# nyuolab/OmniBioTE

Measured on AMD Instinct MI355X. Metric: MLM train tokens/sec, small (8L/1024d) ctx=1024 at 1/2/4/8 MI355X, higher is better.
Workload: dtype bf16

## Files before the change

omnibiote_amd/csrc/elementwise.hip:

```cpp
#include "common.h"
#include <stdlib.h>

namespace {

template <bool INVERSE>
__global__ __launch_bounds__(256) void rope_kernel(bf16* __restrict__ qkv, const float* __restrict__ cos_t,
                                                    const float* __restrict__ sin_t, int64_t rows, int64_t T, int C, int hs) {
    const int chunks_per_row = 2 * C / 8;
    const int64_t total = rows * chunks_per_row;
    for (int64_t i = (int64_t)blockIdx.x * blockDim.x + threadIdx.x; i < total; i += (int64_t)gridDim.x * blockDim.x) {
        const int64_t row = i / chunks_per_row;
        const int col = (int)(i % chunks_per_row) * 8;
        const int d = col % hs;
        const int64_t t = row % T;
        bf16* ptr = qkv + row * 3 * C + col;
        const bf16x8 v = *reinterpret_cast<const bf16x8*>(ptr);
        const f32x4 c = *reinterpret_cast<const f32x4*>(cos_t + t * (hs / 2) + d / 2);
        const f32x4 s = *reinterpret_cast<const f32x4*>(sin_t + t * (hs / 2) + d / 2);
        bf16x8 o;
#pragma unroll
        for (int j = 0; j < 4; ++j) {
            const float xe = bf2f(v[2 * j]), xo = bf2f(v[2 * j + 1]);
            const float sj = INVERSE ? -s[j] : s[j];
            o[2 * j] = f2bf(xe * c[j] - xo * sj);
// ... 20 lines not shown
            for (int jj = 0; jj < 4; ++jj) {
                const uint32_t bits = drop_pair_bits(rk, (uint32_t)(c >> 1) + jj);
#pragma unroll
                for (int e = 0; e < 2; ++e) v[2 * jj + e] = drop_keep_bits(bits, (uint32_t)e, dc) ? f2bf(bf2f(v[2 * jj + e]) * dc.scale) : f2bf(0.f);
            }
        }
        *reinterpret_cast<bf16x8*>(out + r * cols + c) = v;
    }
}

__global__ __launch_bounds__(256) void dropout_kernel(const bf16* in, bf16* out, int64_t n8, int64_t cols, DropCfg dc) {
    for (int64_t i = (int64_t)blockIdx.x * blockDim.x + threadIdx.x; i < n8; i += (int64_t)gridDim.x * blockDim.x) {
        bf16x8 v = reinterpret_cast<const bf16x8*>(in)[i];
        const int64_t row = (i * 8) / cols;
        const uint32_t c = (uint32_t)((i * 8) - row * cols);
        const uint32_t rk = drop_rowkey((uint64_t)row, dc);
        for (int jj = 0; jj < 4; ++jj) {
            const uint32_t bits = drop_pair_bits(rk, (c >> 1) + jj);
#pragma unroll
            for (int e = 0; e < 2; ++e) v[2 * jj + e] = drop_keep_bits(bits, (uint32_t)e, dc) ? f2bf(bf2f(v[2 * jj + e]) * dc.scale) : f2bf(0.f);
        }
        reinterpret_cast<bf16x8*>(out)[i] = v;
    }
}

constexpr int EMB_CHUNK = 32;

template <bool ACC>
__device__ __forceinline__ void embed_store_row(bf16* dst, const float (&acc)[8]) {
    bf16x8 o;
#pragma unroll
    for (int j = 0; j < 8; ++j) o[j] = f2bf(acc[j]);
    if (ACC) {
        const bf16x8 old = *reinterpret_cast<const bf16x8*>(dst);
#pragma unroll
        for (int j = 0; j < 8; ++j) o[j] = f2bf(bf2f(old[j]) + bf2f(o[j]));
    }
    *reinterpret_cast<bf16x8*>(dst) = o;
}
template <bool ACC>
__device__ __forceinline__ void embed_store_row(float* dst, const float (&acc)[8]) {
    f32x4 lo = f32x4{acc[0], acc[1], acc[2], acc[3]}, hi = f32x4{acc[4], acc[5], acc[6], acc[7]};
    if (ACC) {
        lo += *reinterpret_cast<const f32x4*>(dst);
        hi += *reinterpret_cast<const f32x4*>(dst + 4);
    }
    *reinterpret_cast<f32x4*>(dst) = lo;
    *reinterpret_cast<f32x4*>(dst + 4) = hi;
}

template <bool ACC, class DST = bf16>
__global__ __launch_bounds__(128) void embed_bwd_chunk_kernel(const int64_t* __restrict__ idx, const int32_t* __restrict__ order,
                                                               const bf16* __restrict__ dout, DST* __restrict__ dwte,
                                                               float* __restrict__ slab, int64_t rows, int cols, int64_t vocab, DropCfg dc) {
    __shared__ int32_t s_row[EMB_CHUNK];
    __shared__ int64_t s_tok[EMB_CHUNK + 2];
    const int64_t c = blockIdx.x;
    const int64_t p0 = c * EMB_CHUNK;
    const int n = (int)((rows - p0) < EMB_CHUNK ? (rows - p0) : EMB_CHUNK);
    if (threadIdx.x < n) {
        const int32_t r = order[p0 + threadIdx.x];
        s_row[threadIdx.x] = r;
        s_tok[threadIdx.x + 1] = clamp_tok(idx[r], vocab);
    }
    if (threadIdx.x == 64) s_tok[0] = p0 > 0 ? clamp_tok(idx[order[p0 - 1]], vocab) : -1;
    if (threadIdx.x == 65) s_tok[n + 1] = (p0 + n < rows) ? clamp_tok(idx[order[p0 + n]], vocab) : -1;
    __syncthreads();
    const bool left_open = s_tok[0] == s_tok[1];
    const bool right_open = s_tok[n + 1] == s_tok[n];
    for (int col = threadIdx.x * 8; col < cols; col += 128 * 8) {
        float acc[8];
#pragma unroll
        for (int j = 0; j < 8; ++j) acc[j] = 0.f;
        int seg_start = 0;
        for (int i = 0; i < n; ++i) {
            const bf16x8 v = *reinterpret_cast<const bf16x8*>(dout + (int64_t)s_row[i] * cols + col);
            if (dc.thresh16) {
                const uint32_t rk = drop_rowkey((uint64_t)s_row[i], dc);
                for (int jj = 0; jj < 4; ++jj) {
                    const uint32_t bits = drop_pair_bits(rk, (uint32_t)(col >> 1) + jj);
#pragma unroll
                    for (int e = 0; e < 2; ++e)
                        if (drop_keep_bits(bits, (uint32_t)e, dc)) acc[2 * jj + e] += bf2f(f2bf(bf2f(v[2 * jj + e]) * dc.scale));
                }
            } else {
#pragma unroll
                for (int j = 0; j < 8; ++j) acc[j] += bf2f(v[j]);
            }
            const bool seg_end = (i == n - 1) || (s_tok[i + 2] != s_tok[i + 1]);
            if (seg_end) {
                const bool is_first = seg_start == 0, is_last = i == n - 1;
                if ((is_first && left_open) || (is_last && right_open)) {
                    float* dst = slab + ((c * 2 + (is_first ? 0 : 1)) * cols + col);
                    *reinterpret_cast<f32x4*>(dst) = f32x4{acc[0], acc[1], acc[2], acc[3]};
                    *reinterpret_cast<f32x4*>(dst + 4) = f32x4{acc[4], acc[5], acc[6], acc[7]};
                } else {
                    embed_store_row<ACC>(dwte + s_tok[i + 1] * cols + col, acc);
                }
#pragma unroll
                for (int j = 0; j < 8; ++j) acc[j] = 0.f;
                seg_start = i + 1;
            }
        }
    }
}

template <bool ACC, class DST = bf16>
__global__ __launch_bounds__(128) void embed_bwd_span_kernel(const int64_t* __restrict__ idx, const int32_t* __restrict__ order,
                                                              DST* __restrict__ dwte, const float* __restrict__ slab,
                                                              int64_t rows, int cols, int64_t nchunks, int64_t vocab) {
    const int64_t c = blockIdx.x;
    const int64_t p0 = c * EMB_CHUNK;
    const int64_t p1 = (p0 + EMB_CHUNK < rows) ? p0 + EMB_CHUNK : rows;
    const int64_t first = clamp_tok(idx[order[p0]], vocab), last = clamp_tok(idx[order[p1 - 1]], vocab);
    const bool single = first == last;
    const bool left_open = p0 > 0 && clamp_tok(idx[order[p0 - 1]], vocab) == first;
    const bool right_open = p1 < rows && clamp_tok(idx[order[p1]], vocab) == last;
    if (!right_open || (single && left_open)) return;
    const int slot0 = single ? 0 : 1;
    for (int col = threadIdx.x * 8; col < cols; col += 128 * 8) {
        float acc[8];
        const float* src = slab + ((c * 2 + slot0) * cols + col);
#pragma unroll
        for (int j = 0; j < 8; ++j) acc[j] = src[j];
        for (int64_t cc = c + 1; cc < nchunks; ++cc) {
            const int64_t q0 = cc * EMB_CHUNK;
            const int64_t q1 = (q0 + EMB_CHUNK < rows) ? q0 + EMB_CHUNK : rows;
            if (clamp_tok(idx[order[q0]], vocab) != last) break;
            const float* s2 = slab + ((cc * 2) * cols + col);
#pragma unroll
            for (int j = 0; j < 8; ++j) acc[j] += s2[j];
            if (clamp_tok(idx[order[q1 - 1]], vocab) != last) break;
        }
        embed_store_row<ACC>(dwte + last * cols + col, acc);
    }
}

__global__ __launch_bounds__(256) void acc32_add_kernel(float* __restrict__ acc32, const bf16* __restrict__ src, bf16* __restrict__ out,
                                                         int64_t n8, int mode) {
    for (int64_t i = (int64_t)blockIdx.x * 256 + threadIdx.x; i < n8; i += (int64_t)gridDim.x * 256) {
        float v[8];
        if (src) {
            const bf16x8 sv = *reinterpret_cast<const bf16x8*>(src + i * 8);
#pragma unroll
            for (int j = 0; j < 8; ++j) v[j] = bf2f(sv[j]);
        } else {
#pragma unroll
            for (int j = 0; j < 8; ++j) v[j] = 0.f;
        }
        if (mode != OBTE_ACC32_FIRST) {
            const f32x4 lo = *reinterpret_cast<const f32x4*>(acc32 + i * 8), hi = *reinterpret_cast<const f32x4*>(acc32 + i * 8 + 4);
#pragma unroll
            for (int j = 0; j < 4; ++j) { v[j] += lo[j]; v[4 + j] += hi[j]; }
        }
        if (src || mode == OBTE_ACC32_FIRST) {
            *reinterpret_cast<f32x4*>(acc32 + i * 8) = f32x4{v[0], v[1], v[2], v[3]};
            *reinterpret_cast<f32x4*>(acc32 + i * 8 + 4) = f32x4{v[4], v[5], v[6], v[7]};
        }
        if (mode == OBTE_ACC32_LAST) {
            bf16x8 o;
#pragma unroll
            for (int j = 0; j < 8; ++j) o[j] = f2bf(v[j]);
            *reinterpret_cast<bf16x8*>(out + i * 8) = o;
        }
    }
}

__global__ __launch_bounds__(256) void masked_ce_kernel(const bf16* __restrict__ logits, const int64_t* __restrict__ target,
                                                         const uint8_t* __restrict__ mlm_mask, const uint8_t* __restrict__ prev_mask,
                                                         const float* __restrict__ grad_scale, float row_scale,
                                                         float* __restrict__ row_loss, bf16* __restrict__ dlogits, int64_t vocab,
                                                         const int64_t* __restrict__ row_index, const float* __restrict__ row_scale_vec) {
    __shared__ float red[8];
    const int64_t r = blockIdx.x;
    const int64_t src = row_index ? row_index[r] : r;
    const int lane = threadIdx.x & 63, wave = threadIdx.x >> 6;
    bf16* drow = dlogits + r * vocab;
    if (!row_index && mlm_mask && !mlm_mask[r]) {
        if (threadIdx.x == 0 && row_loss) row_loss[r] = 0.f;
        if (prev_mask && !prev_mask[r]) return;
        const bf16x8 z = {};
        for (int64_t c = (int64_t)threadIdx.x * 8; c < vocab; c += 256 * 8) *reinterpret_cast<bf16x8*>(drow + c) = z;
        return;
    }
    const bf16* lrow = logits + src * vocab;
    float m = -INFINITY, l = 0.f;
    for (int64_t c = (int64_t)threadIdx.x * 8; c < vocab; c += 256 * 8) {
// ... 446 lines not shown

extern "C" int obte_embedding_fwd_dropout(const int64_t* idx, const obte_bf16* wte, obte_bf16* out, int64_t rows, int cols,
                                          int64_t vocab, float p, uint64_t seed, obte_stream s) {
    OBTE_REQUIRE(idx && wte && out, "obte_embedding_fwd: null pointer");
    OBTE_REQUIRE(rows >= 0 && cols > 0 && cols % 8 == 0 && vocab > 0, "obte_embedding_fwd: cols must be a multiple of 8");
    if (check_p("obte_embedding_fwd", p)) return OBTE_EINVAL;
    if (rows == 0) return OBTE_OK;
    hipLaunchKernelGGL(embed_fwd_kernel, dim3(stream_grid(rows * (cols / 8), 256)), dim3(256), 0, (hipStream_t)s, idx,
                       (const bf16*)wte, (bf16*)out, rows, cols, vocab, make_drop(p, seed, OBTE_SITE_EMBED));
    OBTE_CHECK_LAUNCH("obte_embedding_fwd");
    return OBTE_OK;
}

extern "C" int obte_embedding_fwd(const int64_t* idx, const obte_bf16* wte, obte_bf16* out, int64_t rows, int cols,
                                  int64_t vocab, obte_stream s) {
    return obte_embedding_fwd_dropout(idx, wte, out, rows, cols, vocab, 0.f, 0, s);
}

__global__ __launch_bounds__(256) void dropout_rows_kernel(const bf16* __restrict__ in, const bf16* __restrict__ aux, bf16* __restrict__ out,
                                                           const int64_t* __restrict__ rows, int64_t n_rows, int cols, DropCfg cfg) {
    const int64_t i = (int64_t)blockIdx.x * 4 + (threadIdx.x >> 6);
    if (i >= n_rows) return;
    const int lane = threadIdx.x & 63;
    const uint32_t rk = drop_rowkey((uint64_t)rows[i], cfg);
    for (int c = lane * 8; c < cols; c += 512) {
        bf16x8 v = *reinterpret_cast<const bf16x8*>(in + i * cols + c);
        bf16x8 a = {};
        if (aux) a = *reinterpret_cast<const bf16x8*>(aux + i * cols + c);
#pragma unroll
        for (int jj = 0; jj < 4; ++jj) {
            const uint32_t bits = drop_pair_bits(rk, ((uint32_t)c >> 1) + jj);
#pragma unroll
            for (int e = 0; e < 2; ++e) {
                const int j = 2 * jj + e;
                const float t = drop_keep_bits(bits, (uint32_t)e, cfg) ? bf2f(f2bf(bf2f(v[j]) * cfg.scale)) : 0.f;
                v[j] = aux ? f2bf(bf2f(a[j]) + t) : f2bf(t);
            }
        }
        *reinterpret_cast<bf16x8*>(out + i * cols + c) = v;
    }
}

extern "C" int obte_dropout_bf16(const obte_bf16* in, obte_bf16* out, int64_t n, int64_t cols, float p, uint64_t seed, int32_t site,
                                 obte_stream s) {
    OBTE_REQUIRE(in && out && n > 0 && n % 8 == 0, "obte_dropout_bf16: null pointer or n not a positive multiple of 8");
    OBTE_REQUIRE(cols > 0 && cols % 8 == 0 && n % cols == 0 && cols < (1ll << 32), "obte_dropout_bf16: cols must be a multiple of 8 that divides n");
    if (check_p("obte_dropout_bf16", p)) return OBTE_EINVAL;
    hipLaunchKernelGGL(dropout_kernel, dim3(stream_grid(n / 8, 256)), dim3(256), 0, (hipStream_t)s, (const bf16*)in, (bf16*)out, n / 8,
                       cols, make_drop(p, seed, (uint32_t)site));
    OBTE_CHECK_LAUNCH("obte_dropout_bf16");
    return OBTE_OK;
}

extern "C" int64_t obte_embedding_bwd_ws_bytes(int64_t rows, int cols) {
    return cdiv64(rows, EMB_CHUNK) * 2 * (int64_t)cols * (int64_t)sizeof(float);
}

extern "C" int obte_embedding_bwd_dropout(const int64_t* idx, const int32_t* order, const obte_bf16* dout, obte_bf16* dwte,
                                          void* ws, int64_t rows, int cols, int64_t vocab, int accumulate, float p, uint64_t seed,
                                          obte_stream s) {
    OBTE_REQUIRE(idx && order && dout && dwte && ws, "obte_embedding_bwd: null pointer");
    if (check_p("obte_embedding_bwd", p)) return OBTE_EINVAL;
    const DropCfg dc = make_drop(p, seed, OBTE_SITE_EMBED);
    OBTE_REQUIRE(rows > 0 && cols > 0 && cols % 8 == 0 && vocab > 0, "obte_embedding_bwd: bad shape");
    OBTE_REQUIRE(rows < (1ll << 31), "obte_embedding_bwd: too many rows");
    hipStream_t st = (hipStream_t)s;
    if (!accumulate && hipMemsetAsync(dwte, 0, (size_t)vocab * cols * sizeof(obte_bf16), st) != hipSuccess) {
        obte_set_error("obte_embedding_bwd: memset failed");
        return OBTE_ELAUNCH;
    }
    const int64_t nchunks = cdiv64(rows, EMB_CHUNK);
    if (accumulate)
        hipLaunchKernelGGL(embed_bwd_chunk_kernel<true>, dim3((unsigned)nchunks), dim3(128), 0, st, idx, order, (const bf16*)dout,
                           (bf16*)dwte, (float*)ws, rows, cols, vocab, dc);
    else
        hipLaunchKernelGGL(embed_bwd_chunk_kernel<false>, dim3((unsigned)nchunks), dim3(128), 0, st, idx, order, (const bf16*)dout,
                           (bf16*)dwte, (float*)ws, rows, cols, vocab, dc);
    OBTE_CHECK_LAUNCH("obte_embedding_bwd(chunk)");
    if (accumulate)
        hipLaunchKernelGGL(embed_bwd_span_kernel<true>, dim3((unsigned)nchunks), dim3(128), 0, st, idx, order, (bf16*)dwte,
                           (const float*)ws, rows, cols, nchunks, vocab);
    else
        hipLaunchKernelGGL(embed_bwd_span_kernel<false>, dim3((unsigned)nchunks), dim3(128), 0, st, idx, order, (bf16*)dwte,
                           (const float*)ws, rows, cols, nchunks, vocab);
    OBTE_CHECK_LAUNCH("obte_embedding_bwd(span)");
    return OBTE_OK;
}

extern "C" int obte_acc32_add_bf16(float* acc32, const obte_bf16* src, obte_bf16* out, int64_t n, int mode, obte_stream s) {
    OBTE_REQUIRE(acc32 && n > 0 && n % 8 == 0, "obte_acc32_add_bf16: null buffer or n not a positive multiple of 8");
    OBTE_REQUIRE(mode >= OBTE_ACC32_FIRST && mode <= OBTE_ACC32_LAST && (mode != OBTE_ACC32_LAST || out), "obte_acc32_add_bf16: bad mode, or LAST without out");
    if (!src && mode == OBTE_ACC32_MORE) return OBTE_OK;
    hipLaunchKernelGGL(acc32_add_kernel, dim3(stream_grid(n / 8, 256)), dim3(256), 0, (hipStream_t)s, acc32, (const bf16*)src, (bf16*)out, n / 8, mode);
    OBTE_CHECK_LAUNCH("obte_acc32_add_bf16");
    return OBTE_OK;
}

extern "C" int obte_embedding_bwd_acc32(const int64_t* idx, const int32_t* order, const obte_bf16* dout, float* acc32, obte_bf16* dwte,
                                        void* ws, int64_t rows, int cols, int64_t vocab, int mode, float p, uint64_t seed, obte_stream s) {
    OBTE_REQUIRE(idx && order && dout && acc32 && ws, "obte_embedding_bwd_acc32: null pointer");
    OBTE_REQUIRE(mode >= OBTE_ACC32_FIRST && mode <= OBTE_ACC32_LAST && (mode != OBTE_ACC32_LAST || dwte), "obte_embedding_bwd_acc32: bad mode, or LAST without dwte");
    if (check_p("obte_embedding_bwd_acc32", p)) return OBTE_EINVAL;
    const DropCfg dc = make_drop(p, seed, OBTE_SITE_EMBED);
    OBTE_REQUIRE(rows > 0 && cols > 0 && cols % 8 == 0 && vocab > 0, "obte_embedding_bwd_acc32: bad shape");
    OBTE_REQUIRE(rows < (1ll << 31), "obte_embedding_bwd_acc32: too many rows");
    hipStream_t st = (hipStream_t)s;
    const bool first = mode == OBTE_ACC32_FIRST;
    if (first && hipMemsetAsync(acc32, 0, (size_t)vocab * cols * sizeof(float), st) != hipSuccess) {
        obte_set_error("obte_embedding_bwd_acc32: memset failed");
        return OBTE_ELAUNCH;
    }
    const int64_t nchunks = cdiv64(rows, EMB_CHUNK);
    if (first)
        hipLaunchKernelGGL((embed_bwd_chunk_kernel<false, float>), dim3((unsigned)nchunks), dim3(128), 0, st, idx, order, (const bf16*)dout, acc32, (float*)ws,
                           rows, cols, vocab, dc);
    else
        hipLaunchKernelGGL((embed_bwd_chunk_kernel<true, float>), dim3((unsigned)nchunks), dim3(128), 0, st, idx, order, (const bf16*)dout, acc32, (float*)ws,
                           rows, cols, vocab, dc);
    OBTE_CHECK_LAUNCH("obte_embedding_bwd_acc32(chunk)");
    if (first)
        hipLaunchKernelGGL((embed_bwd_span_kernel<false, float>), dim3((unsigned)nchunks), dim3(128), 0, st, idx, order, acc32, (const float*)ws, rows, cols,
                           nchunks, vocab);
    else
        hipLaunchKernelGGL((embed_bwd_span_kernel<true, float>), dim3((unsigned)nchunks), dim3(128), 0, st, idx, order, acc32, (const float*)ws, rows, cols,
                           nchunks, vocab);
    OBTE_CHECK_LAUNCH("obte_embedding_bwd_acc32(span)");
    if (mode == OBTE_ACC32_LAST) return obte_acc32_add_bf16(acc32, nullptr, dwte, vocab * (int64_t)cols, OBTE_ACC32_LAST, s);
    return OBTE_OK;
}

extern "C" int obte_embedding_bwd_acc(const int64_t* idx, const int32_t* order, const obte_bf16* dout, obte_bf16* dwte,
                                      void* ws, int64_t rows, int cols, int64_t vocab, int accumulate, obte_stream s) {
    return obte_embedding_bwd_dropout(idx, order, dout, dwte, ws, rows, cols, vocab, accumulate, 0.f, 0, s);
}

extern "C" int obte_embedding_bwd(const int64_t* idx, const int32_t* order, const obte_bf16* dout, obte_bf16* dwte,
                                  void* ws, int64_t rows, int cols, int64_t vocab, obte_stream s) {
    return obte_embedding_bwd_dropout(idx, order, dout, dwte, ws, rows, cols, vocab, 0, 0.f, 0, s);
}

extern "C" int obte_masked_ce_fwd_bwd_reuse(const obte_bf16* logits, const int64_t* target, const uint8_t* mlm_mask,
                                            const uint8_t* prev_mask, const float* grad_scale, float row_scale, float* row_loss,
                                            obte_bf16* dlogits, int64_t rows, int64_t vocab, obte_stream s) {
    OBTE_REQUIRE(logits && target && mlm_mask && grad_scale && dlogits, "obte_masked_ce_fwd_bwd: null pointer");
    OBTE_REQUIRE(rows > 0 && rows < (1ll << 31) && vocab > 0 && vocab % 8 == 0, "obte_masked_ce_fwd_bwd: vocab must be a multiple of 8");
    hipLaunchKernelGGL(masked_ce_kernel, dim3((unsigned)rows), dim3(256), 0, (hipStream_t)s, (const bf16*)logits, target, mlm_mask,
                       prev_mask, grad_scale, row_scale, row_loss, (bf16*)dlogits, vocab, (const int64_t*)nullptr, (const float*)nullptr);
    OBTE_CHECK_LAUNCH("obte_masked_ce_fwd_bwd");
    return OBTE_OK;
}

namespace {
__global__ __launch_bounds__(256) void rows_copy_kernel(const bf16* __restrict__ src, const int64_t* __restrict__ rows, bf16* __restrict__ dst,
                                                         int64_t n_rows, int64_t total_rows, int cols, int scatter) {
    const int wave = threadIdx.x >> 6, lane = threadIdx.x & 63;
    const int64_t i = (int64_t)blockIdx.x * 4 + wave;
    if (i >= n_rows) return;
    int64_t r = rows[i];
    r = r < 0 ? 0 : (r >= total_rows ? total_rows - 1 : r);
    const bf16* s = src + (scatter ? i : r) * cols;
    bf16* d = dst + (scatter ? r : i) * cols;
    for (int c = lane * 8; c < cols; c += 64 * 8) *reinterpret_cast<bf16x8*>(d + c) = *reinterpret_cast<const bf16x8*>(s + c);
}
}
extern "C" int obte_rows_gather_bf16(const obte_bf16* src, const int64_t* rows, obte_bf16* dst, int64_t n_rows, int64_t total_rows, int32_t cols, obte_stream s) {
    OBTE_REQUIRE(src && rows && dst, "obte_rows_gather_bf16: null pointer");
    OBTE_REQUIRE(n_rows > 0 && total_rows > 0 && cols > 0 && cols % 8 == 0, "obte_rows_gather_bf16: need n_rows, total_rows > 0 and cols %% 8 == 0");
    hipLaunchKernelGGL(rows_copy_kernel, dim3((unsigned)cdiv64(n_rows, 4)), dim3(256), 0, (hipStream_t)s, (const bf16*)src, rows, (bf16*)dst, n_rows, total_rows, cols, 0);
    OBTE_CHECK_LAUNCH("obte_rows_gather_bf16");
    return OBTE_OK;
}
extern "C" int obte_rows_scatter_bf16(const obte_bf16* src, const int64_t* rows, obte_bf16* dst, int64_t n_rows, int64_t total_rows, int32_t cols, obte_stream s) {
    OBTE_REQUIRE(src && rows && dst, "obte_rows_scatter_bf16: null pointer");
    OBTE_REQUIRE(n_rows > 0 && n_rows <= total_rows && cols > 0 && cols % 8 == 0, "obte_rows_scatter_bf16: need 0 < n_rows <= total_rows and cols %% 8 == 0");
    if (hipMemsetAsync(dst, 0, (size_t)total_rows * cols * 2, (hipStream_t)s) != hipSuccess) { obte_set_error("obte_rows_scatter_bf16: memset failed"); return OBTE_ELAUNCH; }
    hipLaunchKernelGGL(rows_copy_kernel, dim3((unsigned)cdiv64(n_rows, 4)), dim3(256), 0, (hipStream_t)s, (const bf16*)src, rows, (bf16*)dst, n_rows, total_rows, cols, 1);
    OBTE_CHECK_LAUNCH("obte_rows_scatter_bf16");
    return OBTE_OK;
}
// ... 236 lines not shown
```

omnibiote_amd/csrc/layernorm.hip:

```cpp
#include "common.h"
#include <stdlib.h>

namespace {

constexpr int LN_BWD_MAX_BLOCKS = 512;

template <int NCH, bool FULL>
__global__ __launch_bounds__(256) void ln_fwd_kernel(const bf16* __restrict__ x, const bf16* __restrict__ w,
                                                      bf16* __restrict__ y, float* __restrict__ mean,
                                                      float* __restrict__ rstd, int64_t rows, int cols, float eps) {
    const int wave = __builtin_amdgcn_readfirstlane(threadIdx.x >> 6), lane = threadIdx.x & 63;
    const int64_t row = (int64_t)blockIdx.x * 4 + wave;
    if (row >= rows) return;
    const bf16* xr = x + row * cols;
    float v[NCH][8];
    bf16x8 wq[NCH];
    float sum = 0.f;
    if (FULL) {
        bf16x8 t[NCH];
#pragma unroll
        for (int i = 0; i < NCH; ++i) t[i] = *reinterpret_cast<const bf16x8*>(xr + (lane + 64 * i) * 8);
#pragma unroll
        for (int i = 0; i < NCH; ++i) wq[i] = *reinterpret_cast<const bf16x8*>(w + (lane + 64 * i) * 8);
        __builtin_amdgcn_sched_barrier(0);
#pragma unroll
        for (int i = 0; i < NCH; ++i)
#pragma unroll
            for (int j = 0; j < 8; ++j) { v[i][j] = bf2f(t[i][j]); sum += v[i][j]; }
    } else {
#pragma unroll
        for (int i = 0; i < NCH; ++i) {
            const int c = (lane + 64 * i) * 8;
            if (c < cols) {
                const bf16x8 t = *reinterpret_cast<const bf16x8*>(xr + c);
#pragma unroll
                for (int j = 0; j < 8; ++j) { v[i][j] = bf2f(t[j]); sum += v[i][j]; }
            } else {
#pragma unroll
                for (int j = 0; j < 8; ++j) v[i][j] = 0.f;
            }
        }
    }
    const float mu = (FULL ? wave_sum_dpp(sum) : wave_sum(sum)) / (float)cols;
    float sq = 0.f;
#pragma unroll
    for (int i = 0; i < NCH; ++i) {
        const int c = (lane + 64 * i) * 8;
        if (FULL || c < cols) {
#pragma unroll
            for (int j = 0; j < 8; ++j) { const float d = v[i][j] - mu; sq += d * d; }
        }
    }
    const float rs = 1.0f / sqrtf((FULL ? wave_sum_dpp(sq) : wave_sum(sq)) / (float)cols + eps);
    if (lane == 0) { mean[row] = mu; rstd[row] = rs; }
    bf16* yr = y + row * cols;
#pragma unroll
    for (int i = 0; i < NCH; ++i) {
        const int c = (lane + 64 * i) * 8;
        if (FULL || c < cols) {
            const bf16x8 wv = FULL ? wq[i] : *reinterpret_cast<const bf16x8*>(w + c);
            bf16x8 o;
#pragma unroll
            for (int j = 0; j < 8; ++j) o[j] = f2bf((v[i][j] - mu) * rs * bf2f(wv[j]));
            *reinterpret_cast<bf16x8*>(yr + c) = o;
        }
    }
}

template <int NCH, bool HAS_RESID>
__global__ __launch_bounds__(256) void ln_bwd_kernel(const bf16* __restrict__ dy, const bf16* __restrict__ x,
                                                      const bf16* __restrict__ w, const float* __restrict__ mean,
                                                      const float* __restrict__ rstd, const bf16* __restrict__ dresid,
                                                      bf16* __restrict__ dx, float* __restrict__ ws, int64_t rows, int cols, int ws_accumulate) {
    extern __shared__ __attribute__((aligned(16))) char smem_raw[];
    float* red = reinterpret_cast<float*>(smem_raw);
    const int wave = threadIdx.x >> 6, lane = threadIdx.x & 63;
    float wv[NCH][8], dwacc[NCH][8];
#pragma unroll
    for (int i = 0; i < NCH; ++i) {
        const int c = (lane + 64 * i) * 8;
        bf16x8 t = {};
        if (c < cols) t = *reinterpret_cast<const bf16x8*>(w + c);
#pragma unroll
        for (int j = 0; j < 8; ++j) { wv[i][j] = bf2f(t[j]); dwacc[i][j] = 0.f; }
    }
    const float inv_c = 1.0f / (float)cols;
    for (int64_t row = (int64_t)blockIdx.x * 4 + wave; row < rows; row += (int64_t)gridDim.x * 4) {
        const float mu = mean[row], rs = rstd[row];
        float xh[NCH][8], g[NCH][8];
        bf16x8 res[NCH];
        float s1 = 0.f, s2 = 0.f;
#pragma unroll
        for (int i = 0; i < NCH; ++i) {
            const int c = (lane + 64 * i) * 8;
            res[i] = bf16x8{};
            if (HAS_RESID && c < cols) res[i] = *reinterpret_cast<const bf16x8*>(dresid + row * cols + c);
        }
#pragma unroll
        for (int i = 0; i < NCH; ++i) {
            const int c = (lane + 64 * i) * 8;
            if (c < cols) {
                const bf16x8 tx = *reinterpret_cast<const bf16x8*>(x + row * cols + c);
                const bf16x8 td = *reinterpret_cast<const bf16x8*>(dy + row * cols + c);
#pragma unroll
                for (int j = 0; j < 8; ++j) {
                    const float d = bf2f(td[j]);
                    xh[i][j] = (bf2f(tx[j]) - mu) * rs;
                    g[i][j] = d * wv[i][j];
                    dwacc[i][j] += d * xh[i][j];
                    s1 += g[i][j];
                    s2 += g[i][j] * xh[i][j];
                }
            } else {
#pragma unroll
                for (int j = 0; j < 8; ++j) { xh[i][j] = 0.f; g[i][j] = 0.f; }
            }
        }
        s1 = wave_sum(s1) * inv_c;
        s2 = wave_sum(s2) * inv_c;
#pragma unroll
        for (int i = 0; i < NCH; ++i) {
            const int c = (lane + 64 * i) * 8;
            if (c < cols) {
                bf16x8 o;
#pragma unroll
                for (int j = 0; j < 8; ++j) {
                    float d = rs * (g[i][j] - s1 - xh[i][j] * s2);
                    if (HAS_RESID) d += bf2f(res[i][j]);
                    o[j] = f2bf(d);
                }
                *reinterpret_cast<bf16x8*>(dx + row * cols + c) = o;
            }
        }
    }
#pragma unroll
    for (int i = 0; i < NCH; ++i) {
        const int c = (lane + 64 * i) * 8;
        if (c < cols) {
#pragma unroll
            for (int j = 0; j < 8; ++j) red[wave * cols + c + j] = dwacc[i][j];
        }
    }
    __syncthreads();
    for (int c = threadIdx.x; c < cols; c += 256) {
        const float t = red[c] + red[cols + c] + red[2 * cols + c] + red[3 * cols + c];
        float* dst = ws + (int64_t)blockIdx.x * cols + c;
        *dst = ws_accumulate ? *dst + t : t;
    }
}

template <int NCH, bool HAS_RESID, bool DROP2, bool FULL>
__global__ __launch_bounds__(256) void ln_bwd_pipe_kernel(const bf16* __restrict__ dy, const bf16* __restrict__ x,
                                                           const bf16* __restrict__ w, const float* __restrict__ mean,
                                                           const float* __restrict__ rstd, const bf16* __restrict__ dresid,
                                                           bf16* __restrict__ dx, float* __restrict__ ws, int64_t rows, int cols, int ws_accumulate,
                                                           bf16* __restrict__ dx_drop, DropCfg dc) {
    extern __shared__ __attribute__((aligned(16))) char smem_raw[];
    float* red = reinterpret_cast<float*>(smem_raw);
    const int wave = __builtin_amdgcn_readfirstlane(threadIdx.x >> 6), lane = threadIdx.x & 63;
    float wv[NCH][8], dwacc[NCH][8];
#pragma unroll
    for (int i = 0; i < NCH; ++i) {
        const int c = (lane + 64 * i) * 8;
        bf16x8 t = {};
        if (FULL || c < cols) t = *reinterpret_cast<const bf16x8*>(w + c);
#pragma unroll
        for (int j = 0; j < 8; ++j) { wv[i][j] = bf2f(t[j]); dwacc[i][j] = 0.f; }
    }
    const float inv_c = 1.0f / (float)cols;
    const int64_t stride = (int64_t)gridDim.x * 4;
    int64_t row = (int64_t)blockIdx.x * 4 + wave;
    bf16x8 cx[NCH], cd[NCH], cr[NCH], nx[NCH], nd[NCH], nr[NCH];
    float cmu = 0.f, crs = 0.f, nmu = 0.f, nrs = 0.f;
    auto fetch = [&](int64_t r, bf16x8 (&fx)[NCH], bf16x8 (&fd)[NCH], bf16x8 (&fr)[NCH], float& fmu, float& frs) {
        fmu = mean[r]; frs = rstd[r];
#pragma unroll
        for (int i = 0; i < NCH; ++i) {
            const int c = (lane + 64 * i) * 8;
            fx[i] = bf16x8{}; fd[i] = bf16x8{}; fr[i] = bf16x8{};
            if (FULL || c < cols) {
                if (HAS_RESID) fr[i] = *reinterpret_cast<const bf16x8*>(dresid + r * cols + c);
                fx[i] = *reinterpret_cast<const bf16x8*>(x + r * cols + c);
                fd[i] = *reinterpret_cast<const bf16x8*>(dy + r * cols + c);
            }
        }
    };
    auto process = [&](int64_t r) {
        const float mu = cmu, rs = crs;
        float xh[NCH][8], g[NCH][8];
        float s1 = 0.f, s2 = 0.f;
#pragma unroll
        for (int i = 0; i < NCH; ++i) {
            const int c = (lane + 64 * i) * 8;
            if (FULL || c < cols) {
#pragma unroll
                for (int j = 0; j < 8; ++j) {
                    const float d = bf2f(cd[i][j]);
                    xh[i][j] = (bf2f(cx[i][j]) - mu) * rs;
                    g[i][j] = d * wv[i][j];
                    dwacc[i][j] += d * xh[i][j];
                    s1 += g[i][j];
                    s2 += g[i][j] * xh[i][j];
                }
            } else {
#pragma unroll
                for (int j = 0; j < 8; ++j) { xh[i][j] = 0.f; g[i][j] = 0.f; }
            }
        }
        s1 = (FULL ? wave_sum_dpp(s1) : wave_sum(s1)) * inv_c;
        s2 = (FULL ? wave_sum_dpp(s2) : wave_sum(s2)) * inv_c;
        const uint32_t rk = DROP2 ? drop_rowkey((uint64_t)r, dc) : 0u;
#pragma unroll
        for (int i = 0; i < NCH; ++i) {
            const int c = (lane + 64 * i) * 8;
            if (FULL || c < cols) {
                bf16x8 o;
#pragma unroll
                for (int j = 0; j < 8; ++j) {
                    float d = rs * (g[i][j] - s1 - xh[i][j] * s2);
                    if (HAS_RESID) d += bf2f(cr[i][j]);
                    o[j] = f2bf(d);
                }
                *reinterpret_cast<bf16x8*>(dx + r * cols + c) = o;
                if (DROP2) {
                    bf16x8 od;
#pragma unroll
                    for (int jj = 0; jj < 4; ++jj) {
                        const uint32_t bits = drop_pair_bits(rk, (uint32_t)(c >> 1) + jj);
#pragma unroll
                        for (int e = 0; e < 2; ++e)
                            od[2 * jj + e] = drop_keep_bits(bits, (uint32_t)e, dc) ? f2bf(bf2f(o[2 * jj + e]) * dc.scale) : f2bf(0.f);
                    }
                    *reinterpret_cast<bf16x8*>(dx_drop + r * cols + c) = od;
                }
            }
        }
    };
    if (row < rows) {
        fetch(row, cx, cd, cr, cmu, crs);
        for (; row + stride < rows; row += stride) {
            fetch(row + stride, nx, nd, nr, nmu, nrs);
            __builtin_amdgcn_sched_barrier(0);
            process(row);
#pragma unroll
            for (int i = 0; i < NCH; ++i) { cx[i] = nx[i]; cd[i] = nd[i]; cr[i] = nr[i]; }
            cmu = nmu; crs = nrs;
        }
        process(row);
    }
#pragma unroll
    for (int i = 0; i < NCH; ++i) {
        const int c = (lane + 64 * i) * 8;
        if (FULL || c < cols) {
#pragma unroll
            for (int j = 0; j < 8; ++j) red[wave * cols + c + j] = dwacc[i][j];
        }
    }
    __syncthreads();
    for (int c = threadIdx.x; c < cols; c += 256) {
        const float t = red[c] + red[cols + c] + red[2 * cols + c] + red[3 * cols + c];
        float* dst = ws + (int64_t)blockIdx.x * cols + c;
        *dst = ws_accumulate ? *dst + t : t;
    }
}

__global__ __launch_bounds__(256) void ln_dw_reduce_kernel(const float* __restrict__ ws, bf16* __restrict__ dw, int nblk, int cols, int accumulate) {
    __shared__ float red[8][32];
    const int cl = threadIdx.x & 31, part = threadIdx.x >> 5;
    const int c = blockIdx.x * 32 + cl;
    float s0 = 0.f, s1 = 0.f, s2 = 0.f, s3 = 0.f;
    if (c < cols) {
        int b = part;
        for (; b + 24 < nblk; b += 32) {
            s0 += ws[(int64_t)b * cols + c];
            s1 += ws[(int64_t)(b + 8) * cols + c];
            s2 += ws[(int64_t)(b + 16) * cols + c];
            s3 += ws[(int64_t)(b + 24) * cols + c];
        }
        for (; b < nblk; b += 8) s0 += ws[(int64_t)b * cols + c];
    }
    red[part][cl] = (s0 + s1) + (s2 + s3);
    __syncthreads();
    if (part == 0 && c < cols) {
        float t = 0.f;
#pragma unroll
        for (int i = 0; i < 8; ++i) t += red[i][cl];
        dw[c] = accumulate ? f2bf(bf2f(dw[c]) + bf2f(f2bf(t))) : f2bf(t);
    }
}

int nch_for(int cols) {
    const int chunks = (cols / 8 + 63) / 64;
    if (chunks <= 1) return 1;
    if (chunks <= 2) return 2;
    if (chunks <= 4) return 4;
    if (chunks <= 8) return 8;
    return 16;
}

}

extern "C" int obte_layernorm_bwd_ws_rows(void) { return LN_BWD_MAX_BLOCKS; }

extern "C" int obte_layernorm_fwd(const obte_bf16* x, const obte_bf16* w, obte_bf16* y, float* mean, float* rstd,
                                  int64_t rows, int cols, float eps, obte_stream s) {
    OBTE_REQUIRE(x && w && y && mean && rstd, "obte_layernorm_fwd: null pointer");
    OBTE_REQUIRE(rows >= 0 && cols > 0 && cols % 8 == 0 && cols <= 4096, "obte_layernorm_fwd: cols must be a multiple of 8 and <= 4096 (got %d)", cols);
    if (rows == 0) return OBTE_OK;
    const dim3 grid((unsigned)cdiv64(rows, 4)), block(256);
    hipStream_t st = (hipStream_t)s;
    const int prof = obte_prof_begin(st, 110, rows, cols, 1);
#define LN_FWD(N) do { if (cols == 512 * N) hipLaunchKernelGGL((ln_fwd_kernel<N, true>), grid, block, 0, st, (const bf16*)x, (const bf16*)w, (bf16*)y, mean, rstd, rows, cols, eps); \
                       else hipLaunchKernelGGL((ln_fwd_kernel<N, false>), grid, block, 0, st, (const bf16*)x, (const bf16*)w, (bf16*)y, mean, rstd, rows, cols, eps); } while (0)
    switch (nch_for(cols)) {
        case 1: LN_FWD(1); break;
        case 2: LN_FWD(2); break;
        case 4: LN_FWD(4); break;
        case 8: LN_FWD(8); break;
        default: LN_FWD(16); break;
    }
#undef LN_FWD
    obte_prof_end(prof, st);
    OBTE_CHECK_LAUNCH("obte_layernorm_fwd");
    return OBTE_OK;
}

extern "C" int obte_layernorm_bwd(const obte_bf16* dy, const obte_bf16* x, const obte_bf16* w, const float* mean,
                                  const float* rstd, const obte_bf16* dresid, obte_bf16* dx, obte_bf16* dw, float* ws,
                                  int64_t rows, int cols, obte_stream s) {
    return obte_layernorm_bwd_acc(dy, x, w, mean, rstd, dresid, dx, dw, ws, rows, cols, 0, s);
}

static int ln_bwd_impl(const obte_bf16* dy, const obte_bf16* x, const obte_bf16* w, const float* mean, const float* rstd,
                       const obte_bf16* dresid, obte_bf16* dx, obte_bf16* dw, float* ws, int64_t rows, int cols, int accumulate_dw,
                       int ws_acc, bool reduce, bool clear_tail, obte_stream s, obte_bf16* dx_drop = nullptr, DropCfg dc = DropCfg{0, 0, 0, 1.0f}) {
    OBTE_REQUIRE(dy && x && w && mean && rstd && dx && ws && (dw || !reduce), "obte_layernorm_bwd: null pointer");
    OBTE_REQUIRE(rows > 0 && cols > 0 && cols % 8 == 0 && cols <= 4096, "obte_layernorm_bwd: bad shape rows=%lld cols=%d", (long long)rows, cols);
    struct LnCfg { int blocks_cap, pipe_on; };
    static const LnCfg lcfg = [] {
        LnCfg c;
        const char* e = getenv("OBTE_LN_BLOCKS");
        c.blocks_cap = e ? atoi(e) : 256;
        if (c.blocks_cap < 1 || c.blocks_cap > LN_BWD_MAX_BLOCKS) c.blocks_cap = 256;
        e = getenv("OBTE_LN_PIPE");
        c.pipe_on = (e && e[0] == '0') ? 0 : 1;
        return c;
    }();
    const int blocks_cap = lcfg.blocks_cap;
    const int nblk = (int)(cdiv64(rows, 4) < blocks_cap ? cdiv64(rows, 4) : blocks_cap);
    const dim3 grid(nblk), block(256);
    const size_t smem = (size_t)4 * cols * sizeof(float);
    hipStream_t st = (hipStream_t)s;
    if (clear_tail && nblk < LN_BWD_MAX_BLOCKS &&
        hipMemsetAsync(ws + (size_t)nblk * cols, 0, (size_t)(LN_BWD_MAX_BLOCKS - nblk) * cols * sizeof(float), st) != hipSuccess) {
        obte_set_error("obte_layernorm_bwd_partial: memset failed");
        return OBTE_ELAUNCH;
    }
    const int prof = obte_prof_begin(st, 111, rows, cols, dresid ? 1 : 0);
    const int pipe_on = lcfg.pipe_on;
    const bool drop2 = dx_drop != nullptr && dc.thresh16 != 0;
#define LN_BWD_GO(K, ...) hipLaunchKernelGGL((K), grid, block, smem, st, (const bf16*)dy, (const bf16*)x, (const bf16*)w, mean, rstd, __VA_ARGS__)
#define LN_PIPE(N, R, D, F) LN_BWD_GO((ln_bwd_pipe_kernel<N, R, D, F>), (const bf16*)(R ? dresid : nullptr), (bf16*)dx, ws, rows, cols, ws_acc, (bf16*)(D ? dx_drop : nullptr), dc)
#define LN_PIPE_F(N, R, D) do { if (cols == 512 * N) LN_PIPE(N, R, D, true); else LN_PIPE(N, R, D, false); } while (0)
#define LN_BWD(N)                                                                                                           \
    do {                                                                                                                    \
        if (drop2) {                                                                                                        \
            if (dresid) LN_PIPE_F(N, true, true); else LN_PIPE_F(N, false, true);                                           \
        } else if (pipe_on) {                                                                                               \
            if (dresid) LN_PIPE_F(N, true, false); else LN_PIPE_F(N, false, false);                                         \
        } else {                                                                                                            \
            if (dresid) LN_BWD_GO((ln_bwd_kernel<N, true>), (const bf16*)dresid, (bf16*)dx, ws, rows, cols, ws_acc);        \
            else LN_BWD_GO((ln_bwd_kernel<N, false>), (const bf16*)nullptr, (bf16*)dx, ws, rows, cols, ws_acc);             \
        }                                                                                                                   \
    } while (0)
    switch (nch_for(cols)) {
        case 1: LN_BWD(1); break;
        case 2: LN_BWD(2); break;
        case 4: LN_BWD(4); break;
        case 8: LN_BWD(8); break;
        default: LN_BWD(16); break;
    }
#undef LN_BWD
#undef LN_PIPE_F
#undef LN_PIPE
#undef LN_BWD_GO
    if (!reduce) obte_prof_end(prof, st);
    OBTE_CHECK_LAUNCH("obte_layernorm_bwd");
    if (reduce) {
        hipLaunchKernelGGL(ln_dw_reduce_kernel, dim3((cols + 31) / 32), dim3(256), 0, st, (const float*)ws, (bf16*)dw,
                           ws_acc || clear_tail ? LN_BWD_MAX_BLOCKS : nblk, cols, accumulate_dw);
        obte_prof_end(prof, st);
        OBTE_CHECK_LAUNCH("obte_layernorm_bwd(dw reduce)");
    }
    return OBTE_OK;
}

extern "C" int obte_layernorm_bwd_acc(const obte_bf16* dy, const obte_bf16* x, const obte_bf16* w, const float* mean,
                                      const float* rstd, const obte_bf16* dresid, obte_bf16* dx, obte_bf16* dw, float* ws,
                                      int64_t rows, int cols, int accumulate_dw, obte_stream s) {
    return ln_bwd_impl(dy, x, w, mean, rstd, dresid, dx, dw, ws, rows, cols, accumulate_dw, 0, true, false, s);
}

extern "C" int obte_layernorm_bwd_partial(const obte_bf16* dy, const obte_bf16* x, const obte_bf16* w, const float* mean,
                                          const float* rstd, const obte_bf16* dresid, obte_bf16* dx, obte_bf16* dw, float* partials,
                                          int64_t rows, int cols, int mode, obte_stream s) {
    OBTE_REQUIRE(mode >= OBTE_LN_PARTIAL_FIRST && mode <= OBTE_LN_PARTIAL_LAST, "obte_layernorm_bwd_partial: bad mode %d", mode);
    return ln_bwd_impl(dy, x, w, mean, rstd, dresid, dx, dw, partials, rows, cols, 0, mode != OBTE_LN_PARTIAL_FIRST,
                       mode == OBTE_LN_PARTIAL_LAST, mode == OBTE_LN_PARTIAL_FIRST, s);
}

extern "C" int obte_layernorm_bwd_dropout(const obte_bf16* dy, const obte_bf16* x, const obte_bf16* w, const float* mean,
                                          const float* rstd, const obte_bf16* dresid, obte_bf16* dx, obte_bf16* dx_dropped, obte_bf16* dw,
                                          float* ws_or_partials, int64_t rows, int cols, int partial_mode, int accumulate_dw,
                                          float p, uint64_t seed, int32_t site, obte_stream s) {
    OBTE_REQUIRE(dx_dropped, "obte_layernorm_bwd_dropout: null dx_dropped");
    OBTE_REQUIRE(p >= 0.f && p < 1.f, "obte_layernorm_bwd_dropout: dropout p must be in [0,1)");
    OBTE_REQUIRE(partial_mode == 0 || (partial_mode >= OBTE_LN_PARTIAL_FIRST && partial_mode <= OBTE_LN_PARTIAL_LAST), "obte_layernorm_bwd_dropout: bad partial_mode %d", partial_mode);
    if (p == 0.f) {
        const int rc = partial_mode ? obte_layernorm_bwd_partial(dy, x, w, mean, rstd, dresid, dx, dw, ws_or_partials, rows, cols, partial_mode, s)
                                    : obte_layernorm_bwd_acc(dy, x, w, mean, rstd, dresid, dx, dw, ws_or_partials, rows, cols, accumulate_dw, s);
        if (rc != OBTE_OK) return rc;
        if (hipMemcpyAsync(dx_dropped, dx, (size_t)rows * cols * 2, hipMemcpyDeviceToDevice, (hipStream_t)s) != hipSuccess) {
            obte_set_error("obte_layernorm_bwd_dropout: copy failed");
            return OBTE_ELAUNCH;
        }
// ... 9 lines not shown
```

Baseline: 1.274 million.

## Fuse embedding-backward span merge into chunk kernel; fold LN tail clear into kernel

Replaces the separate embedding-backward span kernel with a last-arriver scheme inside the chunk kernel. Each boundary chunk finds its run extent by galloping binary search, bumps an atomic counter, and the final arriver sums the slab partials with batched loads. The layernorm backward tail memset is moved into the kernel, where each block zeroes the unused workspace rows. This drops one kernel launch per call and one memset per LN backward, but adds a counter memset, atomics and fences to the embedding path.

After: 1.273 million, median of 2. No clear change (-0.1%).

```diff
diff --git a/omnibiote_amd/csrc/elementwise.hip b/omnibiote_amd/csrc/elementwise.hip
--- a/omnibiote_amd/csrc/elementwise.hip
+++ b/omnibiote_amd/csrc/elementwise.hip
@@ -96,7 +96,8 @@
 template <bool ACC, class DST = bf16>
 __global__ __launch_bounds__(128) void embed_bwd_chunk_kernel(const int64_t* __restrict__ idx, const int32_t* __restrict__ order,
                                                                const bf16* __restrict__ dout, DST* __restrict__ dwte,
-                                                               float* __restrict__ slab, int64_t rows, int cols, int64_t vocab, DropCfg dc) {
+                                                               float* __restrict__ slab, unsigned* __restrict__ run_cnt, int64_t rows, int cols,
+                                                               int64_t nchunks, int64_t vocab, DropCfg dc) {
     __shared__ int32_t s_row[EMB_CHUNK];
     __shared__ int64_t s_tok[EMB_CHUNK + 2];
     const int64_t c = blockIdx.x;
@@ -147,36 +148,87 @@
             }
         }
     }
-}
-
-template <bool ACC, class DST = bf16>
-__global__ __launch_bounds__(128) void embed_bwd_span_kernel(const int64_t* __restrict__ idx, const int32_t* __restrict__ order,
-                                                              DST* __restrict__ dwte, const float* __restrict__ slab,
-                                                              int64_t rows, int cols, int64_t nchunks, int64_t vocab) {
-    const int64_t c = blockIdx.x;
-    const int64_t p0 = c * EMB_CHUNK;
-    const int64_t p1 = (p0 + EMB_CHUNK < rows) ? p0 + EMB_CHUNK : rows;
-    const int64_t first = clamp_tok(idx[order[p0]], vocab), last = clamp_tok(idx[order[p1 - 1]], vocab);
-    const bool single = first == last;
-    const bool left_open = p0 > 0 && clamp_tok(idx[order[p0 - 1]], vocab) == first;
-    const bool right_open = p1 < rows && clamp_tok(idx[order[p1]], vocab) == last;
-    if (!right_open || (single && left_open)) return;
-    const int slot0 = single ? 0 : 1;
-    for (int col = threadIdx.x * 8; col < cols; col += 128 * 8) {
-        float acc[8];
-        const float* src = slab + ((c * 2 + slot0) * cols + col);
-#pragma unroll
-        for (int j = 0; j < 8; ++j) acc[j] = src[j];
-        for (int64_t cc = c + 1; cc < nchunks; ++cc) {
-            const int64_t q0 = cc * EMB_CHUNK;
-            const int64_t q1 = (q0 + EMB_CHUNK < rows) ? q0 + EMB_CHUNK : rows;
-            if (clamp_tok(idx[order[q0]], vocab) != last) break;
-            const float* s2 = slab + ((cc * 2) * cols + col);
-#pragma unroll
-            for (int j = 0; j < 8; ++j) acc[j] += s2[j];
-            if (clamp_tok(idx[order[q1 - 1]], vocab) != last) break;
-        }
-        embed_store_row<ACC>(dwte + last * cols + col, acc);
+    if (!left_open && !right_open) return;
+    __shared__ int64_t s_f[2], s_l[2];
+    __shared__ int s_fin[2], s_slot[2];
+    asm volatile("s_waitcnt vmcnt(0)" ::: "memory");
+    __syncthreads();
+    if (threadIdx.x < 2) {
+        const int e = threadIdx.x;
+        const bool single = s_tok[1] == s_tok[n];
+        const bool takes_part = e == 0 ? (left_open || (single && right_open)) : (!single && right_open);
+        int64_t f = c, l = c;
+        int fin = 0, slot = 0;
+        if (takes_part) {
+            const int64_t tok = e == 0 ? s_tok[1] : s_tok[n];
+            auto tok_at = [&](int64_t pos) { return clamp_tok(idx[order[pos]], vocab); };
+            if (e == 0 && left_open) {
+                int64_t hi = c - 1, lo, step = 1;
+                for (;;) {
+                    lo = hi - step;
+                    if (lo < 0) { lo = -1; break; }
+                    if (tok_at(lo * EMB_CHUNK + EMB_CHUNK - 1) != tok) break;
+                    hi = lo; step *= 2;
+                }
+                while (hi - lo > 1) {
+                    const int64_t mid = lo + (hi - lo) / 2;
+                    if (tok_at(mid * EMB_CHUNK + EMB_CHUNK - 1) == tok) hi = mid; else lo = mid;
+                }
+                f = hi;
+            }
+            if (right_open && (e == 1 || single)) {
+                int64_t lo = c + 1, hi, step = 1;
+                for (;;) {
+                    hi = lo + step;
+                    if (hi >= nchunks) { hi = nchunks; break; }
+                    if (tok_at(hi * EMB_CHUNK) != tok) break;
+                    lo = hi; step *= 2;
+                }
+                while (hi - lo > 1) {
+                    const int64_t mid = lo + (hi - lo) / 2;
+                    if (tok_at(mid * EMB_CHUNK) == tok) lo = mid; else hi = mid;
+                }
+                l = lo;
+            }
+            slot = tok_at(f * EMB_CHUNK) == tok ? 0 : 1;
+            __builtin_amdgcn_fence(__ATOMIC_RELEASE, "agent");
+            asm volatile("s_waitcnt vmcnt(0)" ::: "memory");
+            const unsigned before = __hip_atomic_fetch_add(run_cnt + f, 1u, __ATOMIC_RELAXED, __HIP_MEMORY_SCOPE_AGENT);
+            fin = before == (unsigned)(l - f) ? 1 : 0;
+        }
+        s_f[e] = f; s_l[e] = l; s_fin[e] = fin; s_slot[e] = slot;
+    }
+    __syncthreads();
+#pragma unroll
+    for (int e = 0; e < 2; ++e) {
+        if (!s_fin[e]) continue;
+        __builtin_amdgcn_fence(__ATOMIC_ACQUIRE, "agent");
+        const int64_t f = s_f[e], l = s_l[e], tok = e == 0 ? s_tok[1] : s_tok[n];
+        for (int col = threadIdx.x * 8; col < cols; col += 128 * 8) {
+            float acc[8];
+            const float* src = slab + ((f * 2 + s_slot[e]) * cols + col);
+#pragma unroll
+            for (int j = 0; j < 8; ++j) acc[j] = src[j];
+            for (int64_t c0 = f + 1; c0 <= l; c0 += 8) {
+                f32x4 lo[8], hi[8];
+#pragma unroll
+                for (int k = 0; k < 8; ++k) {
+                    const float* s2 = slab + (((c0 + k <= l ? c0 + k : l) * 2) * cols + col);
+                    lo[k] = *reinterpret_cast<const f32x4*>(s2);
+                    hi[k] = *reinterpret_cast<const f32x4*>(s2 + 4);
+                }
+#pragma unroll
+                for (int k = 0; k < 8; ++k) {
+                    const bool in = c0 + k <= l;
+#pragma unroll
+                    for (int j = 0; j < 4; ++j) {
+                        acc[j] = in ? acc[j] + lo[k][j] : acc[j];
+                        acc[4 + j] = in ? acc[4 + j] + hi[k][j] : acc[4 + j];
+                    }
+                }
+            }
+            embed_store_row<ACC>(dwte + tok * cols + col, acc);
+        }
     }
 }
 
@@ -729,8 +781,15 @@
     return OBTE_OK;
 }
 
+static int64_t emb_cnt_bytes(int64_t nchunks) { return (nchunks * (int64_t)sizeof(unsigned) + 255) / 256 * 256; }
+
 extern "C" int64_t obte_embedding_bwd_ws_bytes(int64_t rows, int cols) {
-    return cdiv64(rows, EMB_CHUNK) * 2 * (int64_t)cols * (int64_t)sizeof(float);
+    return cdiv64(rows, EMB_CHUNK) * 2 * (int64_t)cols * (int64_t)sizeof(float) + emb_cnt_bytes(cdiv64(rows, EMB_CHUNK));
+}
+
+static unsigned* emb_clear_counters(void* ws, int64_t nchunks, int cols, hipStream_t st) {
+    unsigned* cnt = reinterpret_cast<unsigned*>((char*)ws + nchunks * 2 * (int64_t)cols * (int64_t)sizeof(float));
+    return hipMemsetAsync(cnt, 0, (size_t)emb_cnt_bytes(nchunks), st) == hipSuccess ? cnt : nullptr;
 }
 
 extern "C" int obte_embedding_bwd_dropout(const int64_t* idx, const int32_t* order, const obte_bf16* dout, obte_bf16* dwte,
@@ -747,20 +806,18 @@
         return OBTE_ELAUNCH;
     }
     const int64_t nchunks = cdiv64(rows, EMB_CHUNK);
+    unsigned* cnt = emb_clear_counters(ws, nchunks, cols, st);
+    if (!cnt) {
+        obte_set_error("obte_embedding_bwd: memset failed");
+        return OBTE_ELAUNCH;
+    }
     if (accumulate)
         hipLaunchKernelGGL(embed_bwd_chunk_kernel<true>, dim3((unsigned)nchunks), dim3(128), 0, st, idx, order, (const bf16*)dout,
-                           (bf16*)dwte, (float*)ws, rows, cols, vocab, dc);
+                           (bf16*)dwte, (float*)ws, cnt, rows, cols, nchunks, vocab, dc);
     else
         hipLaunchKernelGGL(embed_bwd_chunk_kernel<false>, dim3((unsigned)nchunks), dim3(128), 0, st, idx, order, (const bf16*)dout,
-                           (bf16*)dwte, (float*)ws, rows, cols, vocab, dc);
-    OBTE_CHECK_LAUNCH("obte_embedding_bwd(chunk)");
-    if (accumulate)
-        hipLaunchKernelGGL(embed_bwd_span_kernel<true>, dim3((unsigned)nchunks), dim3(128), 0, st, idx, order, (bf16*)dwte,
-                           (const float*)ws, rows, cols, nchunks, vocab);
-    else
-        hipLaunchKernelGGL(embed_bwd_span_kernel<false>, dim3((unsigned)nchunks), dim3(128), 0, st, idx, order, (bf16*)dwte,
-                           (const float*)ws, rows, cols, nchunks, vocab);
-    OBTE_CHECK_LAUNCH("obte_embedding_bwd(span)");
+                           (bf16*)dwte, (float*)ws, cnt, rows, cols, nchunks, vocab, dc);
+    OBTE_CHECK_LAUNCH("obte_embedding_bwd");
     return OBTE_OK;
 }
 
@@ -788,20 +845,18 @@
         return OBTE_ELAUNCH;
     }
     const int64_t nchunks = cdiv64(rows, EMB_CHUNK);
+    unsigned* cnt = emb_clear_counters(ws, nchunks, cols, st);
+    if (!cnt) {
+        obte_set_error("obte_embedding_bwd_acc32: memset failed");
+        return OBTE_ELAUNCH;
+    }
     if (first)
         hipLaunchKernelGGL((embed_bwd_chunk_kernel<false, float>), dim3((unsigned)nchunks), dim3(128), 0, st, idx, order, (const bf16*)dout, acc32, (float*)ws,
-                           rows, cols, vocab, dc);
+                           cnt, rows, cols, nchunks, vocab, dc);
     else
         hipLaunchKernelGGL((embed_bwd_chunk_kernel<true, float>), dim3((unsigned)nchunks), dim3(128), 0, st, idx, order, (const bf16*)dout, acc32, (float*)ws,
-                           rows, cols, vocab, dc);
-    OBTE_CHECK_LAUNCH("obte_embedding_bwd_acc32(chunk)");
-    if (first)
-        hipLaunchKernelGGL((embed_bwd_span_kernel<false, float>), dim3((unsigned)nchunks), dim3(128), 0, st, idx, order, acc32, (const float*)ws, rows, cols,
-                           nchunks, vocab);
-    else
-        hipLaunchKernelGGL((embed_bwd_span_kernel<true, float>), dim3((unsigned)nchunks), dim3(128), 0, st, idx, order, acc32, (const float*)ws, rows, cols,
-                           nchunks, vocab);
-    OBTE_CHECK_LAUNCH("obte_embedding_bwd_acc32(span)");
+                           cnt, rows, cols, nchunks, vocab, dc);
+    OBTE_CHECK_LAUNCH("obte_embedding_bwd_acc32");
     if (mode == OBTE_ACC32_LAST) return obte_acc32_add_bf16(acc32, nullptr, dwte, vocab * (int64_t)cols, OBTE_ACC32_LAST, s);
     return OBTE_OK;
 }
diff --git a/omnibiote_amd/csrc/layernorm.hip b/omnibiote_amd/csrc/layernorm.hip
--- a/omnibiote_amd/csrc/layernorm.hip
+++ b/omnibiote_amd/csrc/layernorm.hip
@@ -4,6 +4,24 @@
 namespace {
 
 constexpr int LN_BWD_MAX_BLOCKS = 512;
+
+struct LnTail {
+    int ws_accumulate;
+    int zero_tail;
+};
+
+__device__ __forceinline__ void ln_dw_partial(float* __restrict__ ws, const float* red, int cols, const LnTail& q) {
+    for (int c = threadIdx.x; c < cols; c += 256) {
+        const float t = red[c] + red[cols + c] + red[2 * cols + c] + red[3 * cols + c];
+        float* dst = ws + (int64_t)blockIdx.x * cols + c;
+        *dst = q.ws_accumulate ? *dst + t : t;
+    }
+    if (q.zero_tail) {
+        const int nblk = (int)gridDim.x;
+        for (int r = (int)blockIdx.x + nblk; r < LN_BWD_MAX_BLOCKS; r += nblk)
+            for (int c = threadIdx.x; c < cols; c += 256) ws[(int64_t)r * cols + c] = 0.f;
+    }
+}
 
 template <int NCH, bool FULL>
 __global__ __launch_bounds__(256) void ln_fwd_kernel(const bf16* __restrict__ x, const bf16* __restrict__ w,
@@ -71,7 +89,7 @@
 __global__ __launch_bounds__(256) void ln_bwd_kernel(const bf16* __restrict__ dy, const bf16* __restrict__ x,
                                                       const bf16* __restrict__ w, const float* __restrict__ mean,
                                                       const float* __restrict__ rstd, const bf16* __restrict__ dresid,
-                                                      bf16* __restrict__ dx, float* __restrict__ ws, int64_t rows, int cols, int ws_accumulate) {
+                                                      bf16* __restrict__ dx, float* __restrict__ ws, int64_t rows, int cols, LnTail q) {
     extern __shared__ __attribute__((aligned(16))) char smem_raw[];
     float* red = reinterpret_cast<float*>(smem_raw);
     const int wave = threadIdx.x >> 6, lane = threadIdx.x & 63;
@@ -142,18 +160,14 @@
         }
     }
     __syncthreads();
-    for (int c = threadIdx.x; c < cols; c += 256) {
-        const float t = red[c] + red[cols + c] + red[2 * cols + c] + red[3 * cols + c];
-        float* dst = ws + (int64_t)blockIdx.x * cols + c;
-        *dst = ws_accumulate ? *dst + t : t;
-    }
+    ln_dw_partial(ws, red, cols, q);
 }
 
 template <int NCH, bool HAS_RESID, bool DROP2, bool FULL>
 __global__ __launch_bounds__(256) void ln_bwd_pipe_kernel(const bf16* __restrict__ dy, const bf16* __restrict__ x,
                                                            const bf16* __restrict__ w, const float* __restrict__ mean,
                                                            const float* __restrict__ rstd, const bf16* __restrict__ dresid,
-                                                           bf16* __restrict__ dx, float* __restrict__ ws, int64_t rows, int cols, int ws_accumulate,
+                                                           bf16* __restrict__ dx, float* __restrict__ ws, int64_t rows, int cols, LnTail q,
                                                            bf16* __restrict__ dx_drop, DropCfg dc) {
     extern __shared__ __attribute__((aligned(16))) char smem_raw[];
     float* red = reinterpret_cast<float*>(smem_raw);
@@ -257,11 +271,7 @@
         }
     }
     __syncthreads();
-    for (int c = threadIdx.x; c < cols; c += 256) {
-        const float t = red[c] + red[cols + c] + red[2 * cols + c] + red[3 * cols + c];
-        float* dst = ws + (int64_t)blockIdx.x * cols + c;
-        *dst = ws_accumulate ? *dst + t : t;
-    }
+    ln_dw_partial(ws, red, cols, q);
 }
 
 __global__ __launch_bounds__(256) void ln_dw_reduce_kernel(const float* __restrict__ ws, bf16* __restrict__ dw, int nblk, int cols, int accumulate) {
@@ -351,16 +361,12 @@
     const dim3 grid(nblk), block(256);
     const size_t smem = (size_t)4 * cols * sizeof(float);
     hipStream_t st = (hipStream_t)s;
-    if (clear_tail && nblk < LN_BWD_MAX_BLOCKS &&
-        hipMemsetAsync(ws + (size_t)nblk * cols, 0, (size_t)(LN_BWD_MAX_BLOCKS - nblk) * cols * sizeof(float), st) != hipSuccess) {
-        obte_set_error("obte_layernorm_bwd_partial: memset failed");
-        return OBTE_ELAUNCH;
-    }
+    const LnTail q{ws_acc, clear_tail ? 1 : 0};
     const int prof = obte_prof_begin(st, 111, rows, cols, dresid ? 1 : 0);
     const int pipe_on = lcfg.pipe_on;
     const bool drop2 = dx_drop != nullptr && dc.thresh16 != 0;
 #define LN_BWD_GO(K, ...) hipLaunchKernelGGL((K), grid, block, smem, st, (const bf16*)dy, (const bf16*)x, (const bf16*)w, mean, rstd, __VA_ARGS__)
-#define LN_PIPE(N, R, D, F) LN_BWD_GO((ln_bwd_pipe_kernel<N, R, D, F>), (const bf16*)(R ? dresid : nullptr), (bf16*)dx, ws, rows, cols, ws_acc, (bf16*)(D ? dx_drop : nullptr), dc)
+#define LN_PIPE(N, R, D, F) LN_BWD_GO((ln_bwd_pipe_kernel<N, R, D, F>), (const bf16*)(R ? dresid : nullptr), (bf16*)dx, ws, rows, cols, q, (bf16*)(D ? dx_drop : nullptr), dc)
 #define LN_PIPE_F(N, R, D) do { if (cols == 512 * N) LN_PIPE(N, R, D, true); else LN_PIPE(N, R, D, false); } while (0)
 #define LN_BWD(N)                                                                                                           \
     do {                                                                                                                    \
@@ -369,8 +375,8 @@
         } else if (pipe_on) {                                                                                               \
             if (dresid) LN_PIPE_F(N, true, false); else LN_PIPE_F(N, false, false);                                         \
         } else {                                                                                                            \
-            if (dresid) LN_BWD_GO((ln_bwd_kernel<N, true>), (const bf16*)dresid, (bf16*)dx, ws, rows, cols, ws_acc);        \
-            else LN_BWD_GO((ln_bwd_kernel<N, false>), (const bf16*)nullptr, (bf16*)dx, ws, rows, cols, ws_acc);             \
+            if (dresid) LN_BWD_GO((ln_bwd_kernel<N, true>), (const bf16*)dresid, (bf16*)dx, ws, rows, cols, q);             \
+            else LN_BWD_GO((ln_bwd_kernel<N, false>), (const bf16*)nullptr, (bf16*)dx, ws, rows, cols, q);                  \
         }                                                                                                                   \
     } while (0)
     switch (nch_for(cols)) {
```
